# xmindflow/TransCeption

Hardware: AMD Instinct MI355X
Metric: images/sec fwd+bwd at 224x224 B=16 per GPU (higher is better)
Workload: dtype bf16; 1 GPU; TransCeption (MSTransception) 224x224 B=16/GPU fwd+bwd+SGD, synthetic Synapse npz slices via the device loader, name-seeded random-init weights; global_batch=16, image_size=224, parallelism=dp1, headline_mode=loader, headline_degraded=False, launch_mode=hipGraph replay

## Files before the change

transception_amd/_lib.py:

```python
from __future__ import annotations

import ctypes as C
import os

from . import _header

HERE = os.path.dirname(os.path.abspath(__file__))
LIB_PATH = os.environ.get("TC_LIB_PATH") or os.path.join(HERE, "libtransception_hip.so")

ABI = _header.load()
SIGNATURES = {name: f.argtypes for name, f in ABI.functions.items()}
K, S = ABI.constants, ABI.structs
POST = _header.load(os.path.join(os.path.dirname(_header.HEADER), "transception_post.h"))

ABI_VERSION = K["TC_ABI_VERSION"]
TC_F32, TC_BF16, TC_F16 = K["TC_F32"], K["TC_BF16"], K["TC_F16"]
ACT_NONE, ACT_HSWISH, ACT_COORD, ACT_SIGMOID = K["TC_ACT_NONE"], K["TC_ACT_HSWISH"], K["TC_ACT_COORD"], K["TC_ACT_SIGMOID"]
ACT_GELU, ACT_SCALE, ACT_RELU = K["TC_ACT_GELU"], K["TC_ACT_SCALE"], K["TC_ACT_RELU"]
FFN_NONE, FFN_LN_A, FFN_LN_B, FFN_EP = K["TC_FFN_NONE"], K["TC_FFN_LN_A"], K["TC_FFN_LN_B"], K["TC_FFN_EP"]
EW_PATCHIFY, EW_DEINTERLEAVE, EW_COPY, EW_MULTI_MAX = K["TC_EW_PATCHIFY"], K["TC_EW_DEINTERLEAVE"], K["TC_EW_COPY"], K["TC_EW_MULTI_MAX"]
TC_AUG_WARP, TC_AUG_LINEAR, TC_AUG_BLUR, TC_AUG_PIECEWISE = K["TC_AUG_WARP"], K["TC_AUG_LINEAR"], K["TC_AUG_BLUR"], K["TC_AUG_PIECEWISE"]
TC_AUG_SKIP, TC_AUG_FROM_RAW = K["TC_AUG_SKIP"], K["TC_AUG_FROM_RAW"]
ATTN_DKV_SPLITS = K["TC_ATTN_DKV_SPLITS"]
TC_METRIC_NO_SOURCE, TC_METRIC_SELECT_WORK_BYTES = K["TC_METRIC_NO_SOURCE"], K["TC_METRIC_SELECT_WORK_BYTES"]
TC_IGNORE_NONE = K["TC_IGNORE_NONE"]
POST_ABI_VERSION = POST.constants["TC_POST_ABI_VERSION"]
TC_CC_LARGEST, TC_CC_MIN_VOXELS = POST.constants["TC_CC_LARGEST"], POST.constants["TC_CC_MIN_VOXELS"]

TcGemm, TcLnFold, TcDwFold, TcDwSeg, TcFfnSeg = S["TcGemm"], S["TcLnFold"], S["TcDwFold"], S["TcDwSeg"], S["TcFfnSeg"]
TcFfnFused, TcFfnBwd, TcEffAtt, TcEwSeg, TcSliceAug = S["TcFfnFused"], S["TcFfnBwd"], S["TcEffAtt"], S["TcEwSeg"], S["TcSliceAug"]


class TcError(RuntimeError):
    pass


class _Lib:
    calls = 0

    def __init__(self, path: str = LIB_PATH):
        if not os.path.exists(path):
            raise TcError(f"{path} is missing: build it with `python -m transception_amd.build` "
                          "(there is no CPU/PyTorch fallback for the TransCeption hot path)")
        self.path = path
        self.cdll = C.CDLL(path)
        for name, f in (*ABI.functions.items(), *POST.functions.items()):
            fn = getattr(self.cdll, name)
            fn.argtypes = f.argtypes
            fn.restype = f.restype
            setattr(self, name, fn if f.query else self._checked(name, fn))
        v = self.cdll.tc_abi_version()
        if v != ABI_VERSION:
            raise TcError(f"ABI mismatch: library {v}, host {ABI_VERSION}")
        v = self.cdll.tc_post_abi_version()
        if v != POST_ABI_VERSION:
            raise TcError(f"post-processing ABI mismatch: library {v}, host {POST_ABI_VERSION}")

    @staticmethod
    def _checked(name, fn):
        def call(*a):
            _Lib.calls += 1
            rc = fn(*a)
            if rc != 0:
                raise TcError(f"{name} failed with status {rc}")
        call.__name__ = name
        return call


_lib = None


def lib() -> _Lib:
    global _lib
    if _lib is None:
        _lib = _Lib()
    return _lib
```

transception_amd/build.py:

```python
from __future__ import annotations

import concurrent.futures as cf
import os
import subprocess
import sys

HERE = os.path.dirname(os.path.abspath(__file__))
CSRC = os.path.join(HERE, "csrc")
LIB = os.path.join(HERE, "libtransception_hip.so")
SOURCES = ["gemm.hip", "norm.hip", "dwconv.hip", "softmax.hip", "attention.hip", "attention_seg.hip", "elementwise.hip", "train.hip", "factoratt.hip", "data.hip", "mixffn.hip", "mixffn_bwd.hip", "effatt.hip", "cbam.hip", "ripm.hip", "linln.hip", "lncls.hip", "legacy.hip", "metrics.hip", "postprocess.hip"]
FLAGS = ["--offload-arch=gfx950", "-O3", "-std=c++17", "-fPIC", "-ffp-contract=fast", "-munsafe-fp-atomics"]


def _hipcc() -> str:
    for c in (os.environ.get("HIPCC"), "/opt/rocm/bin/hipcc", "hipcc"):
        if c and (os.path.isabs(c) and os.path.exists(c) or not os.path.isabs(c)):
            return c
    raise RuntimeError("hipcc not found")


def _stale(target: str, deps) -> bool:
    if not os.path.exists(target):
        return True
    t = os.path.getmtime(target)
    return any(os.path.getmtime(d) > t for d in deps)


def build(force: bool = False, verbose: bool = True) -> str:
    hipcc = _hipcc()
    genv = {k: v for k, v in os.environ.items() if not k.startswith(("TC_ATTN_", "TC_AS_", "TC_DKV_", "TC_DQ_"))}
    for gen in ("gen_attn_asm.py", "gen_dkv_asm.py", "gen_dq_asm.py"):
        r = subprocess.run([sys.executable, os.path.join(CSRC, gen)], capture_output=True, text=True, env=genv)
        if r.returncode != 0:
            raise RuntimeError(f"{gen} failed:\n{r.stderr}")
    headers = [os.path.join(CSRC, "tc_common.h"), os.path.join(HERE, "..", "include", "transception_hip.h"),
               os.path.join(HERE, "..", "include", "transception_post.h")]
    extra = {"attention_seg.hip": [os.path.join(CSRC, "attn_fwd_asm.inc"), os.path.join(CSRC, "attn_dkv_asm.inc"), os.path.join(CSRC, "attn_dq_asm.inc")]}
    objdir = os.path.join(HERE, "build")
    os.makedirs(objdir, exist_ok=True)
    jobs = []
    for src in SOURCES:
        s = os.path.join(CSRC, src)
        o = os.path.join(objdir, src.replace(".hip", ".o"))
        if force or _stale(o, [s] + headers + extra.get(src, [])):
            jobs.append((s, o))

    extra_flags = {"lncls.hip": ["-fno-slp-vectorize"]}

    def compile_one(job):
        s, o = job
        cmd = [hipcc, *FLAGS, *extra_flags.get(os.path.basename(s), []), "-c", s, "-o", o]
        r = subprocess.run(cmd, capture_output=True, text=True)
        if r.returncode != 0:
            raise RuntimeError(f"hipcc failed for {s}:\n{r.stderr}")
        return s

    with cf.ThreadPoolExecutor(max_workers=min(6, max(1, len(jobs)))) as ex:
        for s in ex.map(compile_one, jobs):
            if verbose:
                print(f"[build] compiled {os.path.basename(s)}")
    objs = [os.path.join(objdir, s.replace(".hip", ".o")) for s in SOURCES]
    if force or jobs or _stale(LIB, objs):
        r = subprocess.run([hipcc, "--offload-arch=gfx950", "-shared", "-fPIC", "-o", LIB, *objs], capture_output=True, text=True)
        if r.returncode != 0:
            raise RuntimeError(f"link failed:\n{r.stderr}")
        if verbose:
            print(f"[build] linked {LIB}")
    return LIB


if __name__ == "__main__":
    build(force="--force" in sys.argv)
```

transception_amd/engine.py:

```python
from __future__ import annotations

import ctypes as C
import os
from typing import Callable, Dict, List, Optional, Tuple

import torch

from ._lib import (ATTN_DKV_SPLITS, EW_COPY, EW_DEINTERLEAVE, EW_PATCHIFY, TcEffAtt, TcEwSeg, TcFfnBwd, TcFfnFused, ACT_COORD, ACT_GELU, ACT_HSWISH, ACT_NONE, ACT_SCALE, ACT_SIGMOID, FFN_EP, FFN_LN_A, FFN_LN_B, TC_BF16, TC_F16, TC_F32, TcDwFold, TcDwSeg, TcFfnSeg,
                   TcGemm, TcLnFold, lib)

_DT = {torch.float32: TC_F32, torch.bfloat16: TC_BF16, torch.float16: TC_F16}

PROFILE: Optional[dict] = None


SEG_MARKS = os.environ.get("TC_SEG_MARKS", "")
SEG_LABELS: List[str] = []


def _timed(name: str, flops: float, fn):
    if PROFILE is None:
        fn()
        return
    e0, e1 = torch.cuda.Event(enable_timing=True), torch.cuda.Event(enable_timing=True)
# ... 1610 lines not shown
        return outs

    def sr_gather(self, parts, copy, dst: Var):
        assert dst.data.is_contiguous() and dst.is_whole and len(parts) <= 3
        es = dst.data.element_size()
        src, s_off, s_sb, d_off, d_sb, nb, rows, cols = copy
        assert src.data.is_contiguous() and src.is_whole
        segs = [TcEwSeg(EW_DEINTERLEAVE, 0, _ptr(x.data), dst.data.data_ptr() + off * es, 0, sb, 0, dst.ld, B, Pn, Cc, mult, 0, 0)
                for (x, off, sb, B, Pn, Cc, mult) in parts]
        segs.append(TcEwSeg(EW_COPY, 0, src.data.data_ptr() + s_off * es, dst.data.data_ptr() + d_off * es, s_sb, d_sb, src.ld, dst.ld,
                            nb, rows, cols, 0, 0, 0))
        self._ew_multi(segs)

        def bwd():
            dg = self.grad_of(dst)
            if dg is None:
                return
            segs, late = [], []
            for (x, off, sb, B, Pn, Cc, mult) in parts:
                g, acc = self.wgrad(x)
                if acc:
                    late.append((x, off, sb, B, Pn, Cc, mult))
                    continue
                segs.append(TcEwSeg(EW_DEINTERLEAVE, 1, _ptr(g), dg.data_ptr() + off * es, 0, sb, 0, dst.ld, B, Pn, Cc, mult, 0, 0))
            gt = self._region_grad(src.root, s_off, nb * s_sb)
            segs.append(TcEwSeg(EW_COPY, 1, dg.data_ptr() + d_off * es, gt.data_ptr() + s_off * es, d_sb, s_sb, dst.ld, src.ld,
                                nb, rows, cols, 0, 0, 0))
            self._ew_multi(segs)
            for (x, off, sb, B, Pn, Cc, mult) in late:
                self._write_or_add(x, lambda g_: self.L.tc_sr_deinterleave(_ptr(g_), dg.data_ptr() + off * es, sb, dst.ld, B, Pn, Cc, mult,
                                                                            1, self.dt, self.stream))
        self._rec(bwd)

    def copy_rows(self, src: Var, src_off: int, src_sb: int, dst: Var, dst_off: int, dst_sb: int, nb: int, rows: int, cols: int):
        assert src.data.is_contiguous() and dst.data.is_contiguous() and src.is_whole and dst.is_whole
        es = src.data.element_size()
        self.L.tc_copy3d(src.data.data_ptr() + src_off * es, src_sb, src.ld, dst.data.data_ptr() + dst_off * es, dst_sb, dst.ld,
                         nb, rows, cols, 0, self.dt, self.stream)

        def bwd():
            dg = self.grad_of(dst)
            if dg is None:
                return
            gt = self._region_grad(src.root, src_off, nb * src_sb)
            self.L.tc_copy3d(dg.data_ptr() + dst_off * es, dst_sb, dst.ld, gt.data_ptr() + src_off * es, src_sb, src.ld,
                             nb, rows, cols, 1, self.dt, self.stream)
        self._rec(bwd)

    def sr_deinterleave(self, x: Var, dst: Var, dst_off: int, dst_sb: int, B: int, Pn: int, Cc: int, mult: int):
        assert x.data.is_contiguous() and dst.data.is_contiguous()
        es = x.data.element_size()
        self.L.tc_sr_deinterleave(_ptr(x.data), dst.data.data_ptr() + dst_off * es, dst_sb, dst.ld, B, Pn, Cc, mult, 0, self.dt,
                                  self.stream)

        def bwd():
            dg = self.grad_of(dst)
            if dg is None:
                return
            self._write_or_add(x, lambda g: self.L.tc_sr_deinterleave(_ptr(g), dg.data_ptr() + dst_off * es, dst_sb, dst.ld, B,
                                                                      Pn, Cc, mult, 1, self.dt, self.stream))
        self._rec(bwd)

    def transpose(self, x: Var, nb: int) -> Var:
        R, Cc = x.rows // nb, x.cols
        assert x.data.is_contiguous()
        out = self.new(nb * Cc, R)
        self.L.tc_transpose(_ptr(x.data), _ptr(out.data), nb, R, Cc, self.dt, self.stream)

        def bwd():
            d = self.grad_of(out)
            if d is None:
                return
            assert d.is_contiguous()
            self._write_or_add(x, lambda g: self.L.tc_transpose(_ptr(d), _ptr(g), nb, Cc, R, self.dt, self.stream))
        self._rec(bwd)
        return out

    def stem_im2col(self, img: torch.Tensor, B: int, in_ch: int, H: int, W: int) -> Var:
        Ho, Wo = (H - 1) // 4 + 1, (W - 1) // 4 + 1
        out = self.new(B * Ho * Wo, 148, requires_grad=False)
        self.L.tc_stem_im2col(_ptr(img), _ptr(out.data), 148, B, in_ch, H, W, self.dt, self.stream)
        return out

    def window_rows(self, src: Var, dst: Var, B: int, H: int, W: int, ws: int, ntw: int, off: int, to_map: bool):
        Cc = src.cols
        assert dst.cols == Cc and Cc % 8 == 0
        self.n_launch += 1
        self.L.tc_window_rows(_ptr(src.data), src.ld, _ptr(dst.data), dst.ld, B, H, W, ws, ntw, off, Cc, int(to_map), 0, self.dt, self.stream)

        def bwd():
            d = self.grad_of(dst)
            if d is None or not src.requires_grad:
                return
            if to_map:
                r = src.root
                assert src.is_whole
                if r.grad_t is None:
                    r.grad_t = self._zeros.zeros_like(r.data)
                r.whole_written = True
                g, acc = src.apply_path(r.grad_t), 1
            else:
                g, acc = self.wgrad(src)
            self.n_launch += 1
            self.L.tc_window_rows(_ptr(d), d.stride(0), _ptr(g), g.stride(0), B, H, W, ws, ntw, off, Cc, int(not to_map), acc, self.dt, self.stream)
        self._rec(bwd)

    def dropout(self, x: Var, p: float, seed: torch.Tensor, salt: int) -> Var:
        if not self.training or p <= 0.0:
            return x
        assert x.data.is_contiguous()
        out = self.new(x.rows, x.cols)
        n = x.rows * x.cols
        self.n_launch += 1
        self.L.tc_dropout(_ptr(x.data), _ptr(out.data), n, float(p), _ptr(seed), salt, self.dt, self.stream)

        def bwd():
            d = self.grad_of(out)
            if d is None or not x.requires_grad:
                return
            assert d.is_contiguous()
            tmp = torch.empty_like(d)
            self.L.tc_dropout(_ptr(d), _ptr(tmp), n, float(p), _ptr(seed), salt, self.dt, self.stream)
            self.pass_grad(x, tmp)
        self._rec(bwd)
        return out

    def im2col3s2(self, x, B: int, Cin: int, H: int, W: int, src_ch: int = 0) -> Var:
        Ho, Wo = (H - 1) // 2 + 1, (W - 1) // 2 + 1
        image = not isinstance(x, Var)
        ldc = (9 * Cin + 7) // 8 * 8
        buf = self.new(B * Ho * Wo, ldc, requires_grad=not image)
        self.n_launch += 1
        self.L.tc_im2col3s2(_ptr(x) if image else _ptr(x.data), 0 if image else x.ld, int(image), src_ch if image else 0, _ptr(buf.data), ldc, B, Cin, H, W,
                            self.dt, self.stream)
        cols = buf.colslice(0, 9 * Cin)
        if image:
            return cols

        def bwd():
            d = self.grad_of(cols)
            if d is None or not x.requires_grad:
                return
            gx, acc = self.wgrad(x)
            self.n_launch += 1
            self.L.tc_col2im3s2(_ptr(d), d.stride(0), _ptr(gx), gx.stride(0), B, Cin, H, W, acc, self.dt, self.stream)
        self._rec(bwd)
        return cols

    def im2col_dil(self, x: Var, B: int, H: int, W: int, k: int, stride: int, pad: int, dil: int) -> Var:
        Cin = x.cols
        Ho, Wo = (H + 2 * pad - dil * (k - 1) - 1) // stride + 1, (W + 2 * pad - dil * (k - 1) - 1) // stride + 1
        cols = self.new(B * Ho * Wo, k * k * Cin)
        self.n_launch += 1
        self.L.tc_im2col_dil(_ptr(x.data), x.ld, _ptr(cols.data), cols.ld, B, Cin, H, W, k, stride, pad, dil, self.dt, self.stream)

        def bwd():
            d = self.grad_of(cols)
            if d is None or not x.requires_grad:
                return
            gx, acc = self.wgrad(x)
            self.n_launch += 1
            self.L.tc_col2im_dil(_ptr(d), d.stride(0), _ptr(gx), gx.stride(0), B, Cin, H, W, k, stride, pad, dil, acc, self.dt, self.stream)
        self._rec(bwd)
        return cols

    def nearest_concat(self, seq: Var, B: int, H1: int, W1: int, Ho: int, Wo: int, branch_major: bool = True) -> Var:
# ... 96 lines not shown
```

transception_amd/legacy.py:

```python
from __future__ import annotations

from typing import List

import torch
import torch.nn as nn

from .engine import Graph, Var
from .model import (DIMS, MSTransception, _decoders, _eff_block, _lin, _ln, _mixffn_plain, _mixffn_site, _mk_decoder_layer,
                    _mk_eff_block, _mk_mixffn, _mk_mixffn_skip, _proj_ln, _sk_block)

SIZE = 224
SIDES = (56, 28, 14, 7)


def _branch_geometry(dil_conv) -> tuple:
    if dil_conv:
        return (3, 2, 0, 2), (1, 2, 0, 1)
    return (3, 2, 1, 1), (1, 2, 0, 1)


def _mk_patch_embed(cin: int, cout: int, k: int, stride: int, pad: int, dil: int = 1) -> nn.Module:
    m = nn.Module()
    m.proj = nn.Conv2d(cin, cout, k, stride, pad, dil)
    m.norm = nn.LayerNorm(cout)
# ... 81 lines not shown
            raise ValueError(f"Transception takes 224 x 224 inputs, got {S} x {S}")
        return _forward_legacy(self, G, x, B, in_ch)

    def gradient_pieces(self):
        raise NotImplementedError("Transception: the split backward of the multi-GPU step (gradient_pieces) exists for MSTransception only; "
                                  "train this model with the single-GPU step")


def _patch_embed(M, G: Graph, m: Var, name: str, B: int, side: int, geo, out: Var) -> int:
    k, s, p, d = geo
    Cin = m.cols
    if k == 1 and p == 0:
        W, b = _lin(M, G, name + ".proj")
    else:
        off, shape = M._index[name + ".proj.weight"]
        W = G.permuted_weight(M._P(G, name + ".proj.weight", (shape[0], Cin * k * k)), shape[0], Cin, k * k)
        b = M._P(G, name + ".proj.bias")
    cols = G.im2col_dil(m, B, side, side, k, s, p, d)
    t = G.linear(cols, W, b)
    _ln(M, G, t, name + ".norm", out=out)
    return (side + 2 * p - d * (k - 1) - 1) // s + 1


def _fuse_attention(M, G: Graph, x: Var, name: str, B: int, n1: int, n2: int, heads: int) -> Var:
    C = x.cols
    n = n1 + n2
    hk = C // heads
    xi = G.new(B * n, C)
    G.copy_rows(x, 0, n1 * C, xi, 0, n * C, B, n1, C)
    G.copy_rows(x, B * n1 * C, n2 * C, xi, n1 * C, n * C, B, n2, C)
    kqv = G.new(3 * B * n, C, covered=True)
    Ws = [_lin(M, G, f"{name}.{p}") for p in ("keys", "queries", "values")]
    G.linear_multi(xi, [w for w, _ in Ws], [b for _, b in Ws], kqv, stacked=True)
    K, Q, V = (kqv.rowslice(i * B * n, (i + 1) * B * n).reshape(B * C, n) for i in range(3))
    ksm = G.softmax(K, 1, 1)
    qsm = G.softmax(G.transpose(Q, B).reshape(B * n * heads, hk), 1, 1).reshape(B * n, C)
    ctx = G.new(B * heads * hk, hk)
    G.bmm(ksm, V, ctx, hk, hk, n, 0, 1, nb1=B, nb2=heads, sA=(C * n, hk * n), sB=(C * n, hk * n), sC=(heads * hk * hk, hk * hk))
    o = G.new(B * n, C)
    G.bmm(qsm, ctx, o, n, hk, hk, 0, 0, nb1=B, nb2=heads, sA=(n * C, hk), sB=(heads * hk * hk, hk * hk), sC=(n * C, hk))
    ob = G.new(B * n, C)
    G.copy_rows(o, 0, n * C, ob, 0, n1 * C, B, n1, C)
    G.copy_rows(o, n1 * C, n * C, ob, B * n1 * C, n2 * C, B, n2, C)
    return ob


def _fuse_block(M, G: Graph, x: Var, name: str, B: int, g1: int, g2: int) -> Var:
    n1, n2 = g1 * g1, g2 * g2
    r1 = B * n1
    a = _fuse_attention(M, G, _ln(M, G, x, name + ".norm1"), name + ".attn", B, n1, n2, M.head_count)
    tx, nx = _proj_ln(M, G, a, name + ".attn.reprojection", x, (name + ".norm2", 1e-5))
    out = G.new(x.rows, x.cols)
    parts = [(0, r1, g1, ".mlp1"), (r1, x.rows, g2, ".mlp2")]
    if M.token_mlp_mode == "mix":
        for a0, a1, g, mlp in parts:
            _mixffn_plain(M, G, nx.rowslice(a0, a1), name + mlp, B, g, g, tx.rowslice(a0, a1), out=out.rowslice(a0, a1))
    else:
        G.mixffn([_mixffn_site(M, G, nx.rowslice(a0, a1), name + mlp, B, g, g, tx.rowslice(a0, a1), out.rowslice(a0, a1)) for a0, a1, g, mlp in parts])
    return out


def _inception_stage(M, G: Graph, m: Var, s: int, B: int, side: int) -> Var:
    C = DIMS[s - 1]
    bb = "backbone"
    b1, b2 = _branch_geometry(M.dil_conv)
    g1 = (side + 2 * b1[2] - b1[3] * (b1[0] - 1) - 1) // b1[1] + 1
    g2 = (side + 2 * b2[2] - b2[3] * (b2[0] - 1) - 1) // b2[1] + 1
    assert g2 == SIDES[s - 1]
    r1 = B * g1 * g1
    seq = G.new(r1 + B * g2 * g2, C, covered=True)
    _patch_embed(M, G, m, f"{bb}.patch_embed{s}_1", B, side, b1, seq.rowslice(0, r1))
    _patch_embed(M, G, m, f"{bb}.patch_embed{s}_2", B, side, b2, seq.rowslice(r1, seq.rows))
    for i in range(2):
        seq = _fuse_block(M, G, seq, f"{bb}.block{s}.{i}", B, g1, g2)
    cat = G.nearest_concat(_ln(M, G, seq, f"{bb}.norm{s}"), B, g1, g1, g2, g2, branch_major=True)
    if M.concat == "original":
        return G.linear(cat, *_lin(M, G, f"{bb}.conv1_1_s{s}"))
    return _sk_block(M, G, cat, f"{bb}.sk_concat{s}", B, g2 * g2, C)


def _forward_legacy(M: Transception, G: Graph, x: torch.Tensor, B: int, in_ch: int) -> Var:
    S = SIZE
    G.segment("stage1")
    cols = G.stem_im2col(x, B, in_ch, S, S)
    t = G.linear(cols.colslice(0, 147), *_lin(M, G, "backbone.patch_embed1.proj"))
    t = _ln(M, G, t, "backbone.patch_embed1.norm")
    for i in range(2):
        t = _eff_block(M, G, t, f"backbone.block1.{i}", B, SIDES[0], SIDES[0])
    maps: List[Var] = [_ln(M, G, t, "backbone.norm1")]
    for s in (2, 3, 4):
        G.segment(f"stage{s}")
        maps.append(_inception_stage(M, G, maps[-1], s, B, SIDES[s - 2]))
    G.mark("encoder_done")
    return _decoders(M, G, maps, B, list(SIDES), False)
```

transception_amd/model.py:

```python
from __future__ import annotations

import math
import os
from typing import Dict, List, Optional, Tuple

import torch
import torch.nn as nn

from ._lib import ACT_COORD, ACT_GELU, ACT_HSWISH, ACT_NONE, ACT_RELU, ACT_SIGMOID, TC_BF16, TC_F16, TC_F32, lib
from .engine import Graph, P, Var

DIMS = (64, 128, 320, 512)
LAYERS = (3, 8, 3)
HEADS = 8
CRPE_WINDOW = ((3, 2), (5, 3), (7, 3))
SR_K = (8, 4, 2)
MULT = (1, 2, 5, 8)


def _xavier_convs(mod: nn.Module):
    for m in mod.modules():
        if isinstance(m, nn.Conv2d):
            nn.init.xavier_uniform_(m.weight)
            if m.bias is not None:
# ... 1001 lines not shown
            G.attention(q.rowslice(R[s], R[s + 1]), k, v, B, ntok[s], Nk, Cd ** -0.5, out=att.rowslice(R[s], R[s + 1]))
    return _proj_ln(M, G, att, name + ".proj", X, ln, out=G.new(B * N6, Cd, covered=True), ln_out=G.new(B * N6, Cd, covered=True) if ln is not None else None)


def _bridge_layer(M, G, X: Var, li: int, B: int, sides, ntok, R, N6) -> Var:
    name = f"bridge.bridge_layer{li}"
    n = _ln(M, G, X, name + ".norm1")
    if M.br_ch_att_list[li - 1]:
        tx1 = _channel_att(M, G, n, X, name + ".attn", B, ntok, R, N6)
        tx = _ln(M, G, tx1, name + ".norm2", out=G.new(B * N6, 64, covered=True))
    else:
        tx1, tx = _self_att(M, G, n, X, name + ".attn", B, sides, ntok, R, N6, ln=(name + ".norm2", 1e-5))
    tx2 = G.new(B * N6, 64)
    geo = [(B * sides[s] * sides[s], 64 * MULT[s]) for s in range(4)]
    view = lambda v, s: v.rowslice(R[s], R[s + 1]).reshape(*geo[s])
    G.mixffn([_mixffn_site(M, G, view(tx, s), f"{name}.mixffn{s + 1}", B, sides[s], sides[s], view(tx1, s), view(tx2, s)) for s in range(4)])
    return tx2


def _patch_expand(M, G, t: Var, name: str, B: int, side: int, p: int) -> Var:
    if t.rows != B * side * side:
        raise AssertionError("input feature has wrong size")
    y = G.linear(t, *_lin(M, G, name + ".expand", bias=False))
    return G.layernorm_shuffled(y, M._P(G, name + ".norm.weight"), M._P(G, name + ".norm.bias"), B, side, side, p)


def _decoder(M, G, x1: Var, skip: Var, name: str, B: int, side: int, last: bool) -> Var:
    W, b = _lin(M, G, name + ".concat_linear")
    c1 = x1.cols
    t = G.linear(x1, W, b, wcols=(0, c1))
    G.linear(skip, W, None, out=t, wcols=(c1, c1 + skip.cols), accumulate=True)
    t = _eff_block(M, G, t, name + ".layer_former_1", B, side, side)
    t = _eff_block(M, G, t, name + ".layer_former_2", B, side, side)
    if not last:
        return _patch_expand(M, G, t, name + ".layer_up", B, side, 2)
    tok = bool(getattr(M, "_tok_logits", False))
    up = name + ".layer_up"
    if t.rows != B * side * side:
        raise AssertionError("input feature has wrong size")
    Wc, bc = _lin(M, G, name + ".last_layer")
    gn, bn = M._P(G, up + ".norm.weight"), M._P(G, up + ".norm.bias")
    ye = G.linear(t, *_lin(M, G, up + ".expand", bias=False))
    if G.ln_cls_supported(ye, 4, gn, bn, Wc, bc, B, side, side):
        lg = G.ln_cls(ye, gn, bn, Wc, bc, B, side, side, 4, pad_rows=tok)
    else:
        y = G.layernorm_shuffled(ye, gn, bn, B, side, side, 4)
        lg = G.linear(y, Wc, bc)
    if tok:
        return lg
    return G.transpose(lg, B)


def _forward(M: MSTransception, G: Graph, x: torch.Tensor, B: int, in_ch: int, S: int) -> Var:
    sides = [S // 4, S // 8, S // 16, S // 32]
    ntok = [sides[i] * sides[i] * MULT[i] for i in range(4)]
    N6 = sum(ntok)
    R = [0]
    for nt in ntok:
        R.append(R[-1] + B * nt)
    Xb = G.new(B * N6, 64)

    def stage_map(buf: Var, s: int) -> Var:
        return buf.rowslice(R[s], R[s + 1]).reshape(B * sides[s] * sides[s], 64 * MULT[s])

    tap = getattr(M, "capture_taps", False)
    if M.Stage_3or4 == 4:
        G.segment("stage1")
        m = x
        for i, (cin, hw) in enumerate(((3, S), (DIMS[0] // 2, S // 2))):
            cols = G.im2col3s2(m, B, cin, hw, hw, src_ch=in_ch if i == 0 else 0)
            z = G.linear(cols, *_lin(M, G, f"backbone.stem.{i}.conv", bias=False), bn_shift=_bn_shift(M, f"backbone.stem.{i}.bn"))
            m = _bn(M, G, z, f"backbone.stem.{i}.bn", ACT_HSWISH)
        if tap:
            M.taps = {}
        side = sides[0]
        for s4, (layers, npath) in enumerate(zip((1,) + tuple(LAYERS), (2, 3, 3, 3))):
            if s4 >= 2:
                G.mark(f"stage{s4 + 1}_done")
            G.segment(f"ripm{s4 + 1}")
            stack, side = _ripm(M, G, m, f"backbone.patch_embed_stage{s4 + 1}", B, side, npath, pool=s4 > 0)
            m = _mhca_stage(M, G, stack, f"backbone.mhca_stage{s4 + 1}", layers, B, side, stage_map(Xb, s4), npath)
        return _bridge_and_decoder(M, G, Xb, B, S, sides, ntok, R, N6, tap)
    G.segment("stage1")
    cols = G.stem_im2col(x, B, in_ch, S, S)
    W, b = _lin(M, G, "backbone.patch_embed1.proj")
    t = G.linear(cols.colslice(0, 147), W, b)
    t = _ln(M, G, t, "backbone.patch_embed1.norm")
    if tap:
        M.taps = {"patch_embed1": t.data.float().view(B, sides[0] * sides[0], 64).clone()}
    for i in range(2):
        t = _eff_block(M, G, t, f"backbone.block1.{i}", B, sides[0], sides[0])
    m = _ln(M, G, t, "backbone.norm1", out=stage_map(Xb, 0))
    for s in (1, 2, 3):
        if s >= 2:
            G.mark(f"stage{s + 1}_done")
        G.segment(f"ripm{s + 1}")
        stack, side = _ripm(M, G, m, f"backbone.patch_embed_stage{s + 1}", B, sides[s - 1])
        m = _mhca_stage(M, G, stack, f"backbone.mhca_stage{s + 1}", LAYERS[s - 1], B, side, stage_map(Xb, s))
    return _bridge_and_decoder(M, G, Xb, B, S, sides, ntok, R, N6, tap)


def _spatial_aware_trans(M, G, Xb: Var, name: str, B: int, sides, R, stage_map) -> Var:
    wins, ntw, nb = (8, 4, 2, 1), 85, sides[3]
    assert all(sides[j] == nb * wins[j] for j in range(4)), "SpatialAwareTrans needs the four scales on a common window grid"
    nw, d, h = B * nb * nb, 64, 8
    win = G.new(nw * ntw, d)
    off = 0
    for j in range(4):
        t = G.linear(stage_map(Xb, j), *_lin(M, G, f"{name}.fc{j + 1}"))
        G.window_rows(t, win, B, sides[j], sides[j], wins[j], ntw, off, to_map=False)
        off += wins[j] * wins[j]
    x = win
    seed = M._dropout_seed(G)
    for i in range(M.num_sp):
        blk = f"{name}.group_attention.{i}"
        qkv = G.linear(_ln(M, G, x, blk + ".SlayerNorm_1", 1e-6), *_lin(M, G, blk + ".Attention.qkv_linear"))
        q, k, v = qkv.colslice(0, d), qkv.colslice(d, 2 * d), qkv.colslice(2 * d, 3 * d)
        sc = G.new(nw * h * ntw, ntw)
        G.bmm(q, k, sc, ntw, ntw, d // h, 0, 1, nb1=nw, nb2=h, sA=(ntw * qkv.ld, d // h), sB=(ntw * qkv.ld, d // h), sC=(h * ntw * ntw, ntw * ntw))
        p = G.softmax(sc, 1, 1)
        o = G.new(nw * ntw, d)
        G.bmm(p, v, o, ntw, d // h, ntw, 0, 0, nb1=nw, nb2=h, sA=(h * ntw * ntw, ntw * ntw), sB=(ntw * qkv.ld, d // h), sC=(ntw * d, d // h))
        x = G.linear(o, *_lin(M, G, blk + ".Attention.proj"), residual=x)
        y = G.gelu(G.linear(_ln(M, G, x, blk + ".SlayerNorm_2", 1e-6), *_lin(M, G, blk + ".mlp.fc1")))
        y = G.dropout(y, M.sp_dropout, seed, 2 * i)
        y = G.dropout(G.linear(y, *_lin(M, G, blk + ".mlp.fc2")), M.sp_dropout, seed, 2 * i + 1)
        x = G.add(x, y)
    X = G.new(Xb.rows, Xb.cols)
    off = 0
    for j in range(4):
        t = G.new(B * sides[j] * sides[j], d)
        G.window_rows(x, t, B, sides[j], sides[j], wins[j], ntw, off, to_map=True)
        off += wins[j] * wins[j]
        G.linear(t, *_lin(M, G, f"{name}.fc_back.{j}"), out=stage_map(X, j))
    return X


def _bridge_and_decoder(M: MSTransception, G: Graph, Xb: Var, B: int, S: int, sides, ntok, R, N6: int, tap: bool) -> Var:
    def stage_map(buf: Var, s: int) -> Var:
        return buf.rowslice(R[s], R[s + 1]).reshape(B * sides[s] * sides[s], 64 * MULT[s])

    G.mark("encoder_done")
    X = Xb

    def image_major(buf: Var) -> torch.Tensor:
        return torch.cat([buf.data[R[s]:R[s + 1]].float().view(B, ntok[s], 64) for s in range(4)], dim=1)
    if tap:
        for s in range(4):
            M.taps[f"enc{s}"] = stage_map(Xb, s).data.float().view(B, sides[s], sides[s], 64 * MULT[s]).clone()
    if M.have_bridge == "para":
        b1 = _bridge_layer(M, G, X, 1, B, sides, ntok, R, N6)
        b2 = _bridge_layer(M, G, X, 2, B, sides, ntok, R, N6)
        Wp, bp = _lin(M, G, "bridge.proj_act.0")
        y = G.linear(b1, Wp, bp, wcols=(0, 64))
        G.linear(b2, Wp, None, wcols=(64, 128), out=y, accumulate=True)
        X = _ln(M, G, y, "bridge.proj_act.1", act=ACT_GELU)
        for li in (3, 4):
            X = _bridge_layer(M, G, X, li, B, sides, ntok, R, N6)
        if tap:
            M.taps["bridge4"] = image_major(X)
    elif M.have_bridge != "None":
        if M.have_bridge == "sp" and M.num_sp > 0:
            X = _spatial_aware_trans(M, G, Xb, "bridge.bridge_layer1.scale_fuse_att", B, sides, R, stage_map)
        for li in range(1, 5):
            G.segment(f"bridge{li}")
            X = _bridge_layer(M, G, X, li, B, sides, ntok, R, N6)
            if tap:
                M.taps[f"bridge{li}"] = image_major(X)
    return _decoders(M, G, [stage_map(X, s) for s in range(4)], B, sides, tap)

# ... 15 lines not shown
```

Baseline: 1473 images/sec.

## Fuse stem 7x7 stride-4 conv with LayerNorm and add implicit-GEMM weight gradient

The separate im2col, GEMM and LayerNorm launches for the patch-embed stem are replaced by one MFMA implicit-GEMM kernel. It stages image tiles in LDS, computes the conv plus bias, and writes both the pre-norm and normalized outputs along with the mean and rstd. A matching backward kernel computes the weight and bias gradients straight from the image and upstream gradient, with block-level atomic accumulation. The goal is to avoid writing and re-reading the 147-column im2col matrix and to cut launches, at the cost of custom kernels with limited shape and dtype support and a fallback path.

```diff
diff --git a/include/transception_step.h b/include/transception_step.h
--- /dev/null
+++ b/include/transception_step.h
@@ -0,0 +1,23 @@
+#ifndef TRANSCEPTION_STEP_H
+#define TRANSCEPTION_STEP_H
+
+#ifdef __cplusplus
+extern "C" {
+#endif
+
+#define TC_STEP_ABI_VERSION 1
+#ifndef TC_QUERY
+#define TC_QUERY
+#endif
+
+TC_QUERY int tc_step_abi_version(void);
+TC_QUERY int tc_stem_supported(int in_ch, int dtype);
+int tc_stem_fwd(const void* img, const void* w, const void* b, const void* gamma, const void* beta, void* t, int ldt, void* n, int ldn,
+                float* mean, float* rstd, int B, int in_ch, int H, int W, float eps, int dtype, void* stream);
+int tc_stem_bwd_weight(const void* img, const void* dt, int lddt, float* dw, int lddw, float* db, int B, int in_ch, int H, int W,
+                       int dtype, void* stream);
+
+#ifdef __cplusplus
+}
+#endif
+#endif
diff --git a/transception_amd/_lib.py b/transception_amd/_lib.py
--- a/transception_amd/_lib.py
+++ b/transception_amd/_lib.py
@@ -24,7 +24,9 @@
 ATTN_DKV_SPLITS = K["TC_ATTN_DKV_SPLITS"]
 TC_METRIC_NO_SOURCE, TC_METRIC_SELECT_WORK_BYTES = K["TC_METRIC_NO_SOURCE"], K["TC_METRIC_SELECT_WORK_BYTES"]
 TC_IGNORE_NONE = K["TC_IGNORE_NONE"]
+STEP = _header.load(os.path.join(os.path.dirname(_header.HEADER), "transception_step.h"))
 POST_ABI_VERSION = POST.constants["TC_POST_ABI_VERSION"]
+STEP_ABI_VERSION = STEP.constants["TC_STEP_ABI_VERSION"]
 TC_CC_LARGEST, TC_CC_MIN_VOXELS = POST.constants["TC_CC_LARGEST"], POST.constants["TC_CC_MIN_VOXELS"]
 
 TcGemm, TcLnFold, TcDwFold, TcDwSeg, TcFfnSeg = S["TcGemm"], S["TcLnFold"], S["TcDwFold"], S["TcDwSeg"], S["TcFfnSeg"]
@@ -44,7 +46,7 @@
                           "(there is no CPU/PyTorch fallback for the TransCeption hot path)")
         self.path = path
         self.cdll = C.CDLL(path)
-        for name, f in (*ABI.functions.items(), *POST.functions.items()):
+        for name, f in (*ABI.functions.items(), *POST.functions.items(), *STEP.functions.items()):
             fn = getattr(self.cdll, name)
             fn.argtypes = f.argtypes
             fn.restype = f.restype
@@ -55,6 +57,9 @@
         v = self.cdll.tc_post_abi_version()
         if v != POST_ABI_VERSION:
             raise TcError(f"post-processing ABI mismatch: library {v}, host {POST_ABI_VERSION}")
+        v = self.cdll.tc_step_abi_version()
+        if v != STEP_ABI_VERSION:
+            raise TcError(f"step-kernel ABI mismatch: library {v}, host {STEP_ABI_VERSION}")
 
     @staticmethod
     def _checked(name, fn):
diff --git a/transception_amd/build.py b/transception_amd/build.py
--- a/transception_amd/build.py
+++ b/transception_amd/build.py
@@ -8,7 +8,7 @@
 HERE = os.path.dirname(os.path.abspath(__file__))
 CSRC = os.path.join(HERE, "csrc")
 LIB = os.path.join(HERE, "libtransception_hip.so")
-SOURCES = ["gemm.hip", "norm.hip", "dwconv.hip", "softmax.hip", "attention.hip", "attention_seg.hip", "elementwise.hip", "train.hip", "factoratt.hip", "data.hip", "mixffn.hip", "mixffn_bwd.hip", "effatt.hip", "cbam.hip", "ripm.hip", "linln.hip", "lncls.hip", "legacy.hip", "metrics.hip", "postprocess.hip"]
+SOURCES = ["gemm.hip", "norm.hip", "dwconv.hip", "softmax.hip", "attention.hip", "attention_seg.hip", "elementwise.hip", "train.hip", "factoratt.hip", "data.hip", "mixffn.hip", "mixffn_bwd.hip", "effatt.hip", "cbam.hip", "ripm.hip", "linln.hip", "lncls.hip", "legacy.hip", "metrics.hip", "postprocess.hip", "stem.hip"]
 FLAGS = ["--offload-arch=gfx950", "-O3", "-std=c++17", "-fPIC", "-ffp-contract=fast", "-munsafe-fp-atomics"]
 
 
@@ -34,7 +34,7 @@
         if r.returncode != 0:
             raise RuntimeError(f"{gen} failed:\n{r.stderr}")
     headers = [os.path.join(CSRC, "tc_common.h"), os.path.join(HERE, "..", "include", "transception_hip.h"),
-               os.path.join(HERE, "..", "include", "transception_post.h")]
+               os.path.join(HERE, "..", "include", "transception_post.h"), os.path.join(HERE, "..", "include", "transception_step.h")]
     extra = {"attention_seg.hip": [os.path.join(CSRC, "attn_fwd_asm.inc"), os.path.join(CSRC, "attn_dkv_asm.inc"), os.path.join(CSRC, "attn_dq_asm.inc")]}
     objdir = os.path.join(HERE, "build")
     os.makedirs(objdir, exist_ok=True)
diff --git a/transception_amd/csrc/stem.hip b/transception_amd/csrc/stem.hip
--- /dev/null
+++ b/transception_amd/csrc/stem.hip
@@ -0,0 +1,287 @@
+#include "tc_common.h"
+#include "../../include/transception_step.h"
+
+namespace {
+
+constexpr int ST_TH = 8, ST_TW = 16;
+constexpr int ST_PH = 4 * ST_TH + 3, ST_PW = 4 * ST_TW + 3, ST_PP = ST_PW + 1;
+constexpr int ST_CH = ST_PH * ST_PP;
+constexpr int ST_K = 147, ST_KP = 160, ST_WP = 168;
+constexpr int ST_DP = 72;
+
+struct StemDev {
+    const void *img, *w, *b, *gamma, *beta, *dt;
+    void *t, *n;
+    float *mean, *rstd, *dw, *db;
+    int ldt, ldn, lddt, lddw, B, in_ch, H, W, Ho, Wo, tiles_x, tiles_y, ntiles;
+    float eps;
+};
+
+__device__ __forceinline__ int stem_koff(int k, int in_ch) {
+    if (k >= ST_K) return 0;
+    const int c = k / 49, q = k - c * 49, ky = q / 7, kx = q - ky * 7;
+    return (in_ch == 1 ? 0 : c) * ST_CH + ky * ST_PP + kx;
+}
+
+__device__ __forceinline__ void stem_stage_image(const StemDev& p, unsigned short* im, int b, int ty, int tx) {
+    const unsigned short* src = reinterpret_cast<const unsigned short*>(p.img) + (long long)b * p.in_ch * p.H * p.W;
+    const int iy0 = 4 * ty * ST_TH - 3, ix0 = 4 * tx * ST_TW - 3, n = p.in_ch * (ST_PH * ST_PW);
+    constexpr int U = (ST_PH * ST_PW + 255) / 256;
+    for (int i0 = threadIdx.x; i0 < n; i0 += 256 * U) {
+        unsigned short v[U];
+        int at[U];
+#pragma unroll
+        for (int u = 0; u < U; ++u) {
+            const int i = i0 + 256 * u;
+            const int c = i / (ST_PH * ST_PW), rem = i - c * (ST_PH * ST_PW), py = rem / ST_PW, px = rem - py * ST_PW;
+            const int iy = iy0 + py, ix = ix0 + px;
+            v[u] = 0;
+            at[u] = i < n ? c * ST_CH + py * ST_PP + px : -1;
+            if (i < n && (unsigned)iy < (unsigned)p.H && (unsigned)ix < (unsigned)p.W) v[u] = src[((long long)c * p.H + iy) * p.W + ix];
+        }
+#pragma unroll
+        for (int u = 0; u < U; ++u)
+            if (at[u] >= 0) im[at[u]] = v[u];
+    }
+}
+
+__device__ __forceinline__ void stem_tile_of(const StemDev& p, int tile, int& b, int& ty, int& tx) {
+    const int per = p.tiles_x * p.tiles_y;
+    b = tile / per;
+    const int rem = tile - b * per;
+    ty = rem / p.tiles_x;
+    tx = rem - ty * p.tiles_x;
+}
+
+template <typename T>
+__global__ __launch_bounds__(256) void stem_fwd_kernel(StemDev p) {
+    typedef typename TcHalf<T>::v8 V8;
+    __shared__ __attribute__((aligned(16))) unsigned short im[3 * ST_CH];
+    __shared__ __attribute__((aligned(16))) unsigned short wl[64 * ST_WP];
+    __shared__ __attribute__((aligned(16))) int koff[ST_KP];
+    __shared__ float bs[64], gm[64], bt[64];
+    const int tid = threadIdx.x, lane = tid & 63, wv = tid >> 6, r = lane & 31, h = lane >> 5;
+    {
+        constexpr int NV = 64 * ST_K / 8, U = (NV + 255) / 256;
+        static_assert(NV * 8 == 64 * ST_K, "whole 16-byte pieces");
+        const uint4* w = reinterpret_cast<const uint4*>(p.w);
+        uint4 wv[U];
+#pragma unroll
+        for (int u = 0; u < U; ++u) wv[u] = tid + 256 * u < NV ? w[tid + 256 * u] : make_uint4(0u, 0u, 0u, 0u);
+        for (int i = tid; i < 64 * (ST_WP - ST_K); i += 256) { const int ch = i / (ST_WP - ST_K); wl[ch * ST_WP + ST_K + i - ch * (ST_WP - ST_K)] = 0; }
+#pragma unroll
+        for (int u = 0; u < U; ++u)
+            if (tid + 256 * u < NV) {
+                const unsigned wd[4] = {wv[u].x, wv[u].y, wv[u].z, wv[u].w};
+#pragma unroll
+                for (int e = 0; e < 8; ++e) {
+                    const int i = (tid + 256 * u) * 8 + e, ch = i / ST_K;
+                    wl[ch * ST_WP + i - ch * ST_K] = (unsigned short)(wd[e >> 1] >> (16 * (e & 1)));
+                }
+            }
+        for (int k = tid; k < ST_KP; k += 256) koff[k] = stem_koff(k, p.in_ch);
+        if (tid < 64) {
+            bs[tid] = ldf<T>(reinterpret_cast<const T*>(p.b) + tid);
+            gm[tid] = ldf<T>(reinterpret_cast<const T*>(p.gamma) + tid);
+            bt[tid] = ldf<T>(reinterpret_cast<const T*>(p.beta) + tid);
+        }
+    }
+    const int ly = (wv >> 1) * 4 + (r >> 3), lx = (wv & 1) * 8 + (r & 7);
+    const int base = ly * 4 * ST_PP + lx * 4;
+    for (int tile = blockIdx.x; tile < p.ntiles; tile += gridDim.x) {
+        int b, ty, tx;
+        stem_tile_of(p, tile, b, ty, tx);
+        __syncthreads();
+        stem_stage_image(p, im, b, ty, tx);
+        __syncthreads();
+        tc_f32x16 acc[2];
+#pragma unroll
+        for (int m = 0; m < 2; ++m)
+#pragma unroll
+            for (int i = 0; i < 16; ++i) acc[m][i] = 0.f;
+#pragma unroll
+        for (int s = 0; s < ST_KP / 16; ++s) {
+            const int k0 = 16 * s + 8 * h;
+            const int4 o0 = *reinterpret_cast<const int4*>(koff + k0), o1 = *reinterpret_cast<const int4*>(koff + k0 + 4);
+            uint4 bv;
+            bv.x = (unsigned)im[base + o0.x] | ((unsigned)im[base + o0.y] << 16);
+            bv.y = (unsigned)im[base + o0.z] | ((unsigned)im[base + o0.w] << 16);
+            bv.z = (unsigned)im[base + o1.x] | ((unsigned)im[base + o1.y] << 16);
+            bv.w = (unsigned)im[base + o1.z] | ((unsigned)im[base + o1.w] << 16);
+            const uint4 a0 = *reinterpret_cast<const uint4*>(wl + r * ST_WP + k0);
+            const uint4 a1 = *reinterpret_cast<const uint4*>(wl + (r + 32) * ST_WP + k0);
+            const V8 bf = __builtin_bit_cast(V8, bv);
+            acc[0] = TcHalf<T>::mfma(__builtin_bit_cast(V8, a0), bf, acc[0]);
+            acc[1] = TcHalf<T>::mfma(__builtin_bit_cast(V8, a1), bf, acc[1]);
+        }
+        unsigned tw[16], nw[16];
+        float tv[32], s1 = 0.f;
+#pragma unroll
+        for (int m = 0; m < 2; ++m)
+#pragma unroll
+            for (int i = 0; i < 16; i += 2) {
+                const int ch = 32 * m + 8 * (i >> 2) + 4 * h + (i & 3);
+                const unsigned wd = pack2<T>(acc[m][i] + bs[ch], acc[m][i + 1] + bs[ch + 1]);
+                tw[m * 8 + (i >> 1)] = wd;
+                unpack2<T>(wd, tv[m * 16 + i], tv[m * 16 + i + 1]);
+                s1 += tv[m * 16 + i] + tv[m * 16 + i + 1];
+            }
+        s1 += __shfl_xor(s1, 32, 64);
+        const float mean = s1 * (1.0f / 64);
+        float s2 = 0.f;
+#pragma unroll
+        for (int i = 0; i < 32; ++i) { const float d = tv[i] - mean; s2 += d * d; }
+        s2 += __shfl_xor(s2, 32, 64);
+        const float rstd = rsqrtf(s2 * (1.0f / 64) + p.eps);
+#pragma unroll
+        for (int m = 0; m < 2; ++m)
+#pragma unroll
+            for (int i = 0; i < 16; i += 2) {
+                const int ch = 32 * m + 8 * (i >> 2) + 4 * h + (i & 3);
+                nw[m * 8 + (i >> 1)] = pack2<T>((tv[m * 16 + i] - mean) * rstd * gm[ch] + bt[ch],
+                                                (tv[m * 16 + i + 1] - mean) * rstd * gm[ch + 1] + bt[ch + 1]);
+            }
+        const int oy = ty * ST_TH + ly, ox = tx * ST_TW + lx;
+        const bool live = oy < p.Ho && ox < p.Wo;
+        const long long row = ((long long)b * p.Ho + oy) * p.Wo + ox;
+        T* trow = reinterpret_cast<T*>(p.t) + row * p.ldt;
+        T* nrow = reinterpret_cast<T*>(p.n) + row * p.ldn;
+#pragma unroll
+        for (int j = 0; j < 4; ++j) {
+            const int w0 = 4 * j;
+            const unsigned ts0 = h ? tw[w0] : tw[w0 + 2], ts1 = h ? tw[w0 + 1] : tw[w0 + 3];
+            const unsigned ns0 = h ? nw[w0] : nw[w0 + 2], ns1 = h ? nw[w0 + 1] : nw[w0 + 3];
+            const unsigned tr0 = __shfl_xor(ts0, 32, 64), tr1 = __shfl_xor(ts1, 32, 64);
+            const unsigned nr0 = __shfl_xor(ns0, 32, 64), nr1 = __shfl_xor(ns1, 32, 64);
+            const uint4 to = h ? make_uint4(tr0, tr1, tw[w0 + 2], tw[w0 + 3]) : make_uint4(tw[w0], tw[w0 + 1], tr0, tr1);
+            const uint4 no = h ? make_uint4(nr0, nr1, nw[w0 + 2], nw[w0 + 3]) : make_uint4(nw[w0], nw[w0 + 1], nr0, nr1);
+            if (live) {
+                *reinterpret_cast<uint4*>(trow + 16 * j + 8 * h) = to;
+                *reinterpret_cast<uint4*>(nrow + 16 * j + 8 * h) = no;
+            }
+        }
+        if (live && h == 0) { p.mean[row] = mean; p.rstd[row] = rstd; }
+    }
+}
+
+template <typename T>
+__global__ __launch_bounds__(256) void stem_wgrad_kernel(StemDev p) {
+    typedef typename TcHalf<T>::v8 V8;
+    constexpr int IM = (3 * ST_CH + 7) & ~7;
+    static_assert(2 * (IM + 128 * ST_DP) <= 4 * 64 * ST_KP, "the staged tiles fit inside the buffer they share LDS with");
+    __shared__ __attribute__((aligned(16))) float red[64 * ST_KP];
+    unsigned short* const im = reinterpret_cast<unsigned short*>(red);
+    unsigned short* const dl = im + IM;
+    const int tid = threadIdx.x, lane = tid & 63, wv = tid >> 6, r = lane & 31, h = lane >> 5;
+    const int m = wv & 1, nb0 = (wv >> 1) ? 3 : 0, nnb = (wv >> 1) ? 2 : 3;
+    int ko[3];
+#pragma unroll
+    for (int q = 0; q < 3; ++q) ko[q] = stem_koff(32 * (nb0 + q) + r, p.in_ch);
+    const unsigned one2 = std::is_same<T, bf16_t>::value ? 0x3F803F80u : 0x3C003C00u;
+    const bool ones = (wv >> 1) && r == ST_K - 128;
+    tc_f32x16 acc[3];
+#pragma unroll
+    for (int q = 0; q < 3; ++q)
+#pragma unroll
+        for (int i = 0; i < 16; ++i) acc[q][i] = 0.f;
+    for (int tile = blockIdx.x; tile < p.ntiles; tile += gridDim.x) {
+        int b, ty, tx;
+        stem_tile_of(p, tile, b, ty, tx);
+        __syncthreads();
+        uint4 dv[4];
+#pragma unroll
+        for (int u = 0; u < 4; ++u) {
+            const int i = tid + 256 * u, lp = i >> 3, cq = i & 7, w = lp >> 5, q = lp & 31;
+            const int oy = ty * ST_TH + (w >> 1) * 4 + (q >> 3), ox = tx * ST_TW + (w & 1) * 8 + (q & 7);
+            dv[u] = make_uint4(0u, 0u, 0u, 0u);
+            if (oy < p.Ho && ox < p.Wo)
+                dv[u] = *reinterpret_cast<const uint4*>(reinterpret_cast<const T*>(p.dt) + (((long long)b * p.Ho + oy) * p.Wo + ox) * p.lddt + cq * 8);
+        }
+        stem_stage_image(p, im, b, ty, tx);
+#pragma unroll
+        for (int u = 0; u < 4; ++u) {
+            const int i = tid + 256 * u;
+            *reinterpret_cast<uint4*>(dl + (i >> 3) * ST_DP + (i & 7) * 8) = dv[u];
+        }
+        __syncthreads();
+#pragma unroll
+        for (int st = 0; st < 8; ++st) {
+            const int lp0 = 16 * st + 8 * h;
+            const int rowbase = ((st >> 2) * 4 + 2 * (st & 1) + h) * 4 * ST_PP + ((st >> 1) & 1) * 32;
+            unsigned wa[4];
+#pragma unroll
+            for (int j = 0; j < 8; j += 2)
+                wa[j >> 1] = (unsigned)dl[(lp0 + j) * ST_DP + 32 * m + r] | ((unsigned)dl[(lp0 + j + 1) * ST_DP + 32 * m + r] << 16);
+            const V8 af = __builtin_bit_cast(V8, make_uint4(wa[0], wa[1], wa[2], wa[3]));
+#pragma unroll
+            for (int q = 0; q < 3; ++q)
+                if (q < nnb) {
+                    unsigned wd[4];
+#pragma unroll
+                    for (int j = 0; j < 8; j += 2)
+                        wd[j >> 1] = (unsigned)im[rowbase + 4 * j + ko[q]] | ((unsigned)im[rowbase + 4 * (j + 1) + ko[q]] << 16);
+                    if (q == 1 && ones) { wd[0] = one2; wd[1] = one2; wd[2] = one2; wd[3] = one2; }
+                    acc[q] = TcHalf<T>::mfma(af, __builtin_bit_cast(V8, make_uint4(wd[0], wd[1], wd[2], wd[3])), acc[q]);
+                }
+        }
+    }
+    __syncthreads();
+#pragma unroll
+    for (int q = 0; q < 3; ++q)
+        if (q < nnb) {
+#pragma unroll
+            for (int i = 0; i < 16; ++i) red[(32 * m + 8 * (i >> 2) + 4 * h + (i & 3)) * ST_KP + 32 * (nb0 + q) + r] = acc[q][i];
+        }
+    __syncthreads();
+    for (int i = tid; i < 64 * ST_K; i += 256) {
+        const int ch = i / ST_K, k = i - ch * ST_K;
+        atomicAdd(p.dw + (long long)ch * p.lddw + k, red[ch * ST_KP + k]);
+    }
+    if (p.db && tid < 64) atomicAdd(p.db + tid, red[tid * ST_KP + ST_K]);
+}
+
+bool stem_geometry(StemDev& p, int B, int in_ch, int H, int W) {
+    if (B <= 0 || H <= 0 || W <= 0) return false;
+    p.B = B; p.in_ch = in_ch; p.H = H; p.W = W;
+    p.Ho = (H - 1) / 4 + 1; p.Wo = (W - 1) / 4 + 1;
+    if ((long long)in_ch * H * W >= (1LL << 31) || (long long)B * p.Ho * p.Wo >= (1LL << 31)) return false;
+    p.tiles_x = (p.Wo + ST_TW - 1) / ST_TW; p.tiles_y = (p.Ho + ST_TH - 1) / ST_TH;
+    const long long nt = (long long)B * p.tiles_x * p.tiles_y;
+    if (nt >= (1LL << 31)) return false;
+    p.ntiles = (int)nt;
+    return true;
+}
+
+}
+
+extern "C" int tc_step_abi_version(void) { return TC_STEP_ABI_VERSION; }
+extern "C" int tc_stem_supported(int in_ch, int dtype) { return (dtype == TC_BF16 || dtype == TC_F16) && (in_ch == 1 || in_ch == 3); }
+
+extern "C" int tc_stem_fwd(const void* img, const void* w, const void* b, const void* gamma, const void* beta, void* t, int ldt, void* n, int ldn,
+                           float* mean, float* rstd, int B, int in_ch, int H, int W, float eps, int dtype, void* stream) {
+    if (!img || !w || !b || !gamma || !beta || !t || !n || !mean || !rstd) return TC_ERR_ARG;
+    if (!tc_stem_supported(in_ch, dtype)) return TC_ERR_UNSUPPORTED;
+    StemDev p = {};
+    if (!stem_geometry(p, B, in_ch, H, W)) return TC_ERR_ARG;
+    if (ldt < 64 || ldn < 64 || ldt % 8 || ldn % 8 || (((uintptr_t)t | (uintptr_t)n | (uintptr_t)w) & 15)) return TC_ERR_ARG;
+    p.img = img; p.w = w; p.b = b; p.gamma = gamma; p.beta = beta; p.t = t; p.n = n; p.mean = mean; p.rstd = rstd;
+    p.ldt = ldt; p.ldn = ldn; p.eps = eps;
+    const dim3 grid(p.ntiles < 1024 ? p.ntiles : 1024);
+    if (dtype == TC_BF16) hipLaunchKernelGGL((stem_fwd_kernel<bf16_t>), grid, dim3(256), 0, (hipStream_t)stream, p);
+    else hipLaunchKernelGGL((stem_fwd_kernel<f16_t>), grid, dim3(256), 0, (hipStream_t)stream, p);
+    return tc_launch_status();
+}
+
+extern "C" int tc_stem_bwd_weight(const void* img, const void* dt, int lddt, float* dw, int lddw, float* db, int B, int in_ch, int H, int W,
+                                  int dtype, void* stream) {
+    if (!img || !dt || !dw) return TC_ERR_ARG;
+    if (!tc_stem_supported(in_ch, dtype)) return TC_ERR_UNSUPPORTED;
+    StemDev p = {};
+    if (!stem_geometry(p, B, in_ch, H, W)) return TC_ERR_ARG;
+    if (lddt < 64 || lddt % 8 || ((uintptr_t)dt & 15) || lddw < ST_K) return TC_ERR_ARG;
+    p.img = img; p.dt = dt; p.lddt = lddt; p.dw = dw; p.lddw = lddw; p.db = db;
+    const dim3 grid(p.ntiles < 256 ? p.ntiles : 256);
+    if (dtype == TC_BF16) hipLaunchKernelGGL((stem_wgrad_kernel<bf16_t>), grid, dim3(256), 0, (hipStream_t)stream, p);
+    else hipLaunchKernelGGL((stem_wgrad_kernel<f16_t>), grid, dim3(256), 0, (hipStream_t)stream, p);
+    return tc_launch_status();
+}
diff --git a/transception_amd/engine.py b/transception_amd/engine.py
--- a/transception_amd/engine.py
+++ b/transception_amd/engine.py
@@ -1716,6 +1716,34 @@
         self.L.tc_stem_im2col(_ptr(img), _ptr(out.data), 148, B, in_ch, H, W, self.dt, self.stream)
         return out
 
+    def stem_supported(self, img: torch.Tensor, W: P, b: Optional[P], g: P, beta: P, in_ch: int) -> bool:
+        return (self.dt != TC_F32 and self.ngroups == 1 and b is not None and img.dtype == self.dtype and img.is_contiguous()
+                and W.data.is_contiguous() and tuple(W.data.shape) == (64, 147) and (W.grad is None) == (b.grad is None)
+                and all(q.data.data_ptr() % 16 == 0 for q in (W, b, g, beta)) and bool(self.L.tc_stem_supported(in_ch, self.dt)))
+
+    def stem(self, img: torch.Tensor, W: P, b: P, g: P, beta: P, B: int, in_ch: int, H: int, Wd: int, eps: float = 1e-5) -> Var:
+        Ho, Wo = (H - 1) // 4 + 1, (Wd - 1) // 4 + 1
+        rows = B * Ho * Wo
+        t = self.new(rows, 64)
+        es = t.data.element_size()
+
+        def bwd():
+            dt = self.grad_of(t)
+            if dt is None or W.grad is None:
+                return
+            self.n_launch += 1
+            _timed("hbm:stem_bwd_weight (7x7 s4 conv weight + bias gradient from the image, one launch)", 1.0 * rows * 64 * es + img.numel() * es,
+                   lambda: self.L.tc_stem_bwd_weight(_ptr(img), _ptr(dt), dt.stride(0), _ptr(W.grad), W.grad.stride(0),
+                                                     _ptr(b.grad) if b.grad is not None else None, B, in_ch, H, Wd, self.dt, self.stream))
+        self._rec(bwd)
+        mean, rstd = self.f32(rows), self.f32(rows)
+        xn = self.layernorm(t, g, beta, eps, stats=(mean, rstd), launch=False)
+        self.n_launch += 1
+        _timed("hbm:stem_fwd (7x7 s4 conv + LayerNorm, one launch)", 2.0 * rows * 64 * es + img.numel() * es, lambda: self.L.tc_stem_fwd(
+            _ptr(img), _ptr(W.data), _ptr(b.data), _ptr(g.data), _ptr(beta.data), _ptr(t.data), t.ld, _ptr(xn.data), xn.ld, _ptr(mean), _ptr(rstd),
+            B, in_ch, H, Wd, eps, self.dt, self.stream))
+        return xn
+
     def window_rows(self, src: Var, dst: Var, B: int, H: int, W: int, ws: int, ntw: int, off: int, to_map: bool):
         Cc = src.cols
         assert dst.cols == Cc and Cc % 8 == 0
diff --git a/transception_amd/legacy.py b/transception_amd/legacy.py
--- a/transception_amd/legacy.py
+++ b/transception_amd/legacy.py
@@ -187,9 +187,13 @@
 def _forward_legacy(M: Transception, G: Graph, x: torch.Tensor, B: int, in_ch: int) -> Var:
     S = SIZE
     G.segment("stage1")
-    cols = G.stem_im2col(x, B, in_ch, S, S)
-    t = G.linear(cols.colslice(0, 147), *_lin(M, G, "backbone.patch_embed1.proj"))
-    t = _ln(M, G, t, "backbone.patch_embed1.norm")
+    W, b = _lin(M, G, "backbone.patch_embed1.proj")
+    g, beta = M._P(G, "backbone.patch_embed1.norm.weight"), M._P(G, "backbone.patch_embed1.norm.bias")
+    if G.stem_supported(x, W, b, g, beta, in_ch):
+        t = G.stem(x, W, b, g, beta, B, in_ch, S, S)
+    else:
+        cols = G.stem_im2col(x, B, in_ch, S, S)
+        t = G.layernorm(G.linear(cols.colslice(0, 147), W, b), g, beta)
     for i in range(2):
         t = _eff_block(M, G, t, f"backbone.block1.{i}", B, SIDES[0], SIDES[0])
     maps: List[Var] = [_ln(M, G, t, "backbone.norm1")]
diff --git a/transception_amd/model.py b/transception_amd/model.py
--- a/transception_amd/model.py
+++ b/transception_amd/model.py
@@ -1107,10 +1107,13 @@
             m = _mhca_stage(M, G, stack, f"backbone.mhca_stage{s4 + 1}", layers, B, side, stage_map(Xb, s4), npath)
         return _bridge_and_decoder(M, G, Xb, B, S, sides, ntok, R, N6, tap)
     G.segment("stage1")
-    cols = G.stem_im2col(x, B, in_ch, S, S)
     W, b = _lin(M, G, "backbone.patch_embed1.proj")
-    t = G.linear(cols.colslice(0, 147), W, b)
-    t = _ln(M, G, t, "backbone.patch_embed1.norm")
+    g, beta = M._P(G, "backbone.patch_embed1.norm.weight"), M._P(G, "backbone.patch_embed1.norm.bias")
+    if G.stem_supported(x, W, b, g, beta, in_ch):
+        t = G.stem(x, W, b, g, beta, B, in_ch, S, S)
+    else:
+        cols = G.stem_im2col(x, B, in_ch, S, S)
+        t = G.layernorm(G.linear(cols.colslice(0, 147), W, b), g, beta)
     if tap:
         M.taps = {"patch_embed1": t.data.float().view(B, sides[0] * sides[0], 64).clone()}
     for i in range(2):
```

Measured after the change: 1484 images/sec, median of 2. Within noise of the previous version (+0.7%).
